# oleg-savchenko/jax_nbody_emulator_with_dj

Measured on AMD Instinct MI355X. Metric: voxels/sec (disp+vel) on 512^3 box, ndiv=4, higher is better.
Workload: dtype f32-equivalent: f16x3 split MFMA (3 f16 MFMAs per product, f32 accumulate)

## Files before the change

### jax_nbody_emulator_with_dj_amd/csrc/nbe_engine.cpp

```cpp

#include "../../include/nbe.h"
#include "nbe_kernels.h"

#include <sched.h>

#include <cmath>
#include <cstdarg>
#include <cstdio>
#include <cstdlib>
#include <cstring>
#include <algorithm>
#include <atomic>
#include <chrono>
#include <condition_variable>
#include <deque>
#include <map>
#include <memory>
#include <mutex>
#include <string>
#include <thread>
#include <vector>

using namespace nbe;

// ... 1239 lines not shown
    if (d.k != 3) return fail("%s/%s: conv layers have k=3", d.block, d.layer);
    *kind = 0;
    return 0;
}

static int expected_shape(nbe_ctx* c, const std::string& blk, const std::string& lay, int* cout, int* cin) {
    const int m = c->mid;
    int bi, bo;
    if (blk == "conv_l00") { bi = c->in_chan; bo = m; }
    else if (blk == "conv_r2" || blk == "conv_r1" || blk == "conv_r00") { bi = 2 * m; bo = m; }
    else if (blk == "conv_r01") { bi = m; bo = c->out_chan; }
    else { bi = m; bo = m; }
    const int midc = bi > bo ? bi : bo;
    if (lay == "skip") { *cin = bi; *cout = bo; }
    else if (blk.rfind("down_", 0) == 0 || blk.rfind("up_", 0) == 0) { *cin = bi; *cout = bo; }
    else if (lay == "conv_0") { *cin = bi; *cout = midc; }
    else if (lay == "conv_1") { *cin = midc; *cout = bo; }
    else return fail("unknown layer %s/%s", blk.c_str(), lay.c_str());
    return 0;
}

static const char* kBlocks[15] = {"conv_l00", "conv_l01", "down_l0", "conv_l1", "down_l1", "conv_l2", "down_l2", "conv_c",
                                  "up_r2", "conv_r2", "up_r1", "conv_r1", "up_r0", "conv_r00", "conv_r01"};

static int pack_wino(nbe_ctx* c) {
    c->wino_ok = false;
    if (!((c->prec == PREC_F16X3 && (c->vel ? c->gauge_active : true)) || (c->prec == PREC_F16 && c->vel && c->gauge_active))) return 0;
    if (!c->wino_flag) HIPCHK(hipMalloc((void**)&c->wino_flag, 4));
    HIPCHK(hipMemsetAsync(c->wino_flag, 0, 4, c->stream));
    for (auto& kv : c->layers) {
        Layer& L = kv.second;
        if (L.pw.ww && L.kind == 0 && (L.g6 || !c->vel)) launch_pack_h3w(L.wn, L.cout, L.cin, L.pw.cin_pad, L.pw.ctiles, L.pw.ww, c->wino_flag, c->stream, c->prec);
        if (L.pw.ww && L.kind == 1 && (c->vel ? (L.b_sub && c->fuse) : c->novel_fuse)) {
            launch_pack_h3w_skip(L.wn, L.cout, L.cin, L.pw, L.pw.ww, c->wino_flag, c->stream);
            if (c->vel) launch_pack_h3w_skip(c->prec == PREC_F16 ? L.dwn_f : L.dwn, L.cout, L.cin, L.pw, L.pw.ww + L.pw.floats, c->wino_flag, c->stream);
        }
    }
    int bad = 0;
    HIPCHK(hipMemcpyAsync(&bad, c->wino_flag, 4, hipMemcpyDeviceToHost, c->stream));
    HIPCHK(hipStreamSynchronize(c->stream));
    c->wino_ok = bad == 0;
    if (!c->vel) c->fuse = c->novel_fuse && c->wino_ok;
    if (c->prec == PREC_F16) c->fuse = c->fuse && c->wino_ok;
    return 0;
}

static int wire_novel(nbe_ctx* c) {
    c->novel_fuse = false;
    if (c->vel || c->prec != PREC_F16X3) return 0;
    for (const char* b : kBlocks) {
        if (!strncmp(b, "down_", 5) || !strncmp(b, "up_", 3)) continue;
        auto i1 = c->layers.find(std::string(b) + "/conv_1"), is = c->layers.find(std::string(b) + "/skip");
        if (i1 == c->layers.end() || is == c->layers.end()) return fail("internal: block %s", b);
        Layer &L1 = i1->second, &Ls = is->second;
        if (!L1.pw.ww || !Ls.pw.ww || 2 * (Ls.pw.cin_pad / 16) > 16 || L1.pw.ctiles != Ls.pw.ctiles) return 0;
    }
    for (const char* b : kBlocks) {
        if (!strncmp(b, "down_", 5) || !strncmp(b, "up_", 3)) continue;
        Layer &L1 = c->layers[std::string(b) + "/conv_1"], &Ls = c->layers[std::string(b) + "/skip"];
        L1.fskip = &Ls;
        const int nb = L1.pw.ctiles * 32 * L1.pw.ni;
        HIPCHK(hipMalloc((void**)&L1.bias_f, nb * 4));
    }
    c->novel_fuse = true;
    return 0;
}

static int wire_gauge(nbe_ctx* c) {
// ... 162 lines not shown
        int ec, ei;
        if (expected_shape(c, L.block, L.layer, &ec, &ei)) return 1;
        if (ec != d.cout || ei != d.cin)
            return fail("%s/%s: weight shape (%d,%d,k) does not match the architecture (%d,%d,k)", d.block, d.layer, d.cout, d.cin, ec, ei);
        L.first = (L.block == "conv_l00") && (L.layer == "conv_0" || L.layer == "skip");
        const size_t nw = (size_t)d.cout * d.cin * d.k * d.k * d.k;
        PackedW& pw = L.pw;
        pw.mode = L.kind == 0 ? MODE_FLAT3 : (L.kind == 2 ? MODE_DOWN : MODE_FLAT1);
        pw.prec = c->prec;
        pw.ni = (prec_is_half(c->prec) || d.cout > 32) ? 2 : 1;
        pw.cin = d.cin; pw.cout = d.cout;
        pw.cin_pad = roundup(d.cin, prec_ck(c->prec, pw.mode));
        pw.ctiles = (d.cout + 32 * pw.ni - 1) / (32 * pw.ni);
        pw.nsets = L.kind == 3 ? 8 : 1;
        pw.floats = (int64_t)pw.ctiles * 32 * pw.ni * mode_nseg(pw.mode) * mode_taps(pw.mode) * pw.cin_pad / (c->prec == PREC_F16 ? 2 : 1);
        HIPCHK(hipMalloc((void**)&pw.w, pw.floats * pw.nsets * 4));
        if (c->vel) HIPCHK(hipMalloc((void**)&pw.dw, pw.floats * pw.nsets * 4));
        const int nb = pw.ctiles * 32 * pw.ni;
        HIPCHK(hipMalloc((void**)&pw.bias, nb * 4));
        HIPCHK(hipMemset(pw.bias, 0, nb * 4));
        HIPCHK(hipMemcpy(pw.bias, d.bias, d.cout * 4, hipMemcpyHostToDevice));
        if (c->prec == PREC_F16X3 && c->vel && (L.kind == 0 || L.kind == 1) && d.cout <= 4 && !L.first) {
            PackedW& pn = L.pwn;
            pn = pw; pn.w = nullptr; pn.dw = nullptr;
            pn.cout_t = 16; pn.ctiles = 1;
            pn.floats = (int64_t)16 * mode_nseg(pn.mode) * mode_taps(pn.mode) * pn.cin_pad;
            HIPCHK(hipMalloc((void**)&pn.w, pn.floats * 4));
            if (L.kind == 1) HIPCHK(hipMalloc((void**)&pn.dw, pn.floats * 4));
        }
        if ((c->prec == PREC_F16X3 && L.kind == 0 && !L.first && !L.pwn.w && pw.cin_pad / 16 <= 8) ||
            (L.kind == 0 && !L.first && wino_f16_layer(c->prec, c->vel, pw.cin_pad)))
            HIPCHK(hipMalloc((void**)&pw.ww, pw.floats * 4 / 3 * 4));
        if (c->prec == PREC_F16X3 && L.kind == 1 && !L.pwn.w && pw.cin_pad / 16 <= 8)
            HIPCHK(hipMalloc((void**)&pw.ww, pw.floats * 2 * 4));
        if (style && L.kind == 1 && !L.first && wino_f16_layer(c->prec, c->vel, pw.cin_pad)) {
            HIPCHK(hipMalloc((void**)&pw.ww, pw.floats * 2 * 4));
            HIPCHK(hipMalloc((void**)&L.dwn_f, nw * 4));
        }
        if (prec_is_half(c->prec) && L.kind == 0 && L.first && d.cin <= 3 && d.cout <= 64)
            HIPCHK(hipMalloc((void**)&pw.stem, 4 * 3 * 4 * 64 * 16));
        HIPCHK(hipMalloc((void**)&L.bias0, nb * 4));
        HIPCHK(hipMemcpy(L.bias0, pw.bias, nb * 4, hipMemcpyDeviceToDevice));
        for (int i = 0; i < d.cout; ++i)
            if (std::isfinite(d.bias[i])) c->bias_max = std::max(c->bias_max, std::fabs(d.bias[i]));
        HIPCHK(hipMalloc((void**)&L.wn, nw * 4));
        if (c->vel) HIPCHK(hipMalloc((void**)&L.dwn, nw * 4));
        if (style) {
            if (!d.style_weight || !d.style_bias) return fail("%s/%s: style_weight and style_bias are required", d.block, d.layer);
            HIPCHK(hipMalloc((void**)&L.weight, nw * 4));
            HIPCHK(hipMalloc((void**)&L.sw, d.cin * 2 * 4));
            HIPCHK(hipMalloc((void**)&L.sb, d.cin * 4));
            HIPCHK(hipMemcpy(L.weight, d.weight, nw * 4, hipMemcpyHostToDevice));
            HIPCHK(hipMemcpy(L.sw, d.style_weight, d.cin * 2 * 4, hipMemcpyHostToDevice));
            HIPCHK(hipMemcpy(L.sb, d.style_bias, d.cin * 4, hipMemcpyHostToDevice));
        } else {
            if (c->vel && !d.dweight) return fail("%s/%s: dweight is required for premodulated velocity weights", d.block, d.layer);
            HIPCHK(hipMemcpy(L.wn, d.weight, nw * 4, hipMemcpyHostToDevice));
            if (c->vel) HIPCHK(hipMemcpy(L.dwn, d.dweight, nw * 4, hipMemcpyHostToDevice));
            launch_pack(L.wn, d.cout, d.cin, L.kind, pw, pw.w, c->stream);
            if (c->vel) launch_pack(L.dwn, d.cout, d.cin, L.kind, pw, pw.dw, c->stream);
            if (L.pwn.w) launch_pack(L.wn, d.cout, d.cin, L.kind, L.pwn, L.pwn.w, c->stream);
            if (L.pwn.dw) launch_pack(L.dwn, d.cout, d.cin, L.kind, L.pwn, L.pwn.dw, c->stream);
        }
        c->layers[L.block + "/" + L.layer] = L;
    }
    for (const char* b : kBlocks) {
        const bool rs = !strncmp(b, "down_", 5) || !strncmp(b, "up_", 3);
// ... 1217 lines not shown
```

### jax_nbody_emulator_with_dj_amd/csrc/nbe_kernels.h

```cpp
#pragma once
#include <hip/hip_runtime.h>
#include <stdint.h>

namespace nbe {

struct Planes {
    float* x = nullptr;
    float* dx = nullptr;
    int64_t pstride = 0;
    int G = 0;
    int D = 0, H = 0, W = 0;
    int64_t vox() const { return (int64_t)D * H * W; }
};

enum Precision { PREC_F32 = 0, PREC_F16X3 = 1, PREC_F16 = 2 };
inline constexpr bool prec_is_half(int prec) { return prec == PREC_F16X3 || prec == PREC_F16; }
inline constexpr int prec_parts(int prec) { return prec == PREC_F16X3 ? 2 : 1; }
constexpr float H3_SCALE = 2048.0f, H3_INV = 1.0f / 2048.0f;
constexpr int H3_RANGE_UP = 6;

constexpr int NBE_MAX_GROUPS = 64;

enum ConvMode { MODE_FLAT3 = 0, MODE_FLAT1 = 1, MODE_DOWN = 2 };
enum ConvFlags { F_ACT = 1, F_RES = 2, F_SKIP_NODX = 4 };
// ... 24 lines not shown
    Planes in;
    int64_t in_off = 0;
    int Dv = 0, Hv = 0, Wv = 0;
    Planes out;
    int out_g0 = 0;
    int osz = 1, oz = 0, oy = 0, ox = 0;
    Planes res;
    int flags = 0;
    int set = 0;
    const float* gout = nullptr;
    const float* beta = nullptr;
    const float* bias = nullptr;
    Planes in2;
    int csplit_ch = 0;
    Planes sk, sk2;
    int sk_split_ch = 0;
    int64_t sk_off = 0;
    const PackedW* skw = nullptr;
    bool wino = false;
};

int launch_conv(const PackedW& pw, const ConvLaunch& L, bool vel, bool has_dx, hipStream_t s);

void launch_modulate(const float* weight, const float* style_weight, const float* style_bias,
                     int cout, int cin, int k3, float s0, float s1, float eps, int first_layer,
                     float* w_n, float* dw_tot , hipStream_t s,
                     const float* a_in = nullptr, float* beta_out = nullptr, const float* b_sub = nullptr);
void launch_style_alpha(const float* style_weight, const float* style_bias, int cin, float s0, float s1,
                        float* alpha, int* flag, hipStream_t s);
void launch_pack(const float* w_oidhw, int cout, int cin, int kind, const PackedW& pw, float* dst, hipStream_t s);

void launch_pack_h3w(const float* w_oidhw, int cout, int cin, int cin_pad, int ctiles, float* dst, int* flag, hipStream_t s,
                     int prec = PREC_F16X3);
void launch_pack_h3w_skip(const float* w_oidhw, int cout, int cin, const PackedW& pw, float* dst, int* flag, hipStream_t s);

void launch_gather(const float* box, int C, int Db, int Hb, int Wb, int a0, int a1, int a2,
                   const Planes& dst, float scale, int prec, hipStream_t s);
void launch_to_planes(const float* src, int C, const Planes& dst, bool tangent, float scale, int prec, hipStream_t s);
void launch_from_planes(const Planes& src, bool tangent, int C, float* dst, int prec, hipStream_t s);
void launch_crop(const Planes& src, int c, const Planes& dst, int g0, bool vel, hipStream_t s, int cz = -1);
struct HeadScale { float k_disp = 6.f, k_dy = 0.f, k_x0 = 0.f; int* bad = nullptr; };
void launch_head(const Planes& y, const Planes& xin, int c0, int C, const HeadScale& hs, bool vel,
                 void* disp, void* velo, int out_dtype, int Db, int Hb, int Wb, int a0, int a1, int a2,
                 int prec, hipStream_t s, int pad = 0);
void launch_absmax(const float* src, int64_t n, unsigned* out_bits, hipStream_t s);
void launch_zero(void* dst, int64_t bytes, hipStream_t s);
void launch_scale(const float* src, float* dst, int n, float f, hipStream_t s, const float* src2 = nullptr);

void launch_fill_yx(const Planes& t, int pad, bool vel, hipStream_t s);
void launch_wrap_pad(const Planes& src, const Planes& dst, int pad, bool vel, hipStream_t s, int padz = 0);

void launch_tag_word(unsigned* dst, unsigned v, const unsigned* expect_at, unsigned* flag, unsigned bit, hipStream_t s);

struct ProbeLaunch {
    const float* x; int64_t pstride; int H, W, g0, prec, C;
    int ext[3], org[3], per[3];
    int zlo, zhi, zper;
    int o[3], n, nw;
    unsigned* bits; unsigned* count;
};
void launch_probe_signs(const ProbeLaunch& a, hipStream_t s);

void h3q_read_stamps(double* out16, hipStream_t s);

}
```

### jax_nbody_emulator_with_dj_amd/csrc/nbe_kernels_h3.hip

```cpp

#include "nbe_kernels_internal.h"
#include <cstdlib>
#include <cstdio>
#include <algorithm>

#ifndef NBE_DBG
#define NBE_DBG 0
#endif

namespace nbe {

extern __shared__ __attribute__((aligned(16))) f32x4 lds_h3[];

__device__ __forceinline__ void split4(const f32x4 v, half4& hi, half4& lo) {
#pragma unroll
    for (int e = 0; e < 4; ++e) {
        hi[e] = (_Float16)v[e];
        lo[e] = (_Float16)__builtin_fmaf((float)hi[e], -H3_SCALE, v[e] * H3_SCALE);
    }
}
__device__ __forceinline__ f32x4 join4(const half4 hi, const half4 lo) {
    f32x4 v;
#pragma unroll
    for (int e = 0; e < 4; ++e) v[e] = (float)hi[e] + (float)lo[e] * H3_INV;
// ... 1825 lines not shown
    const int nstage = nseg * nchunk;
    long r = idx;
    const int j = (int)(r % 8); r /= 8;
    const int co = (int)(r % cout_t); r /= cout_t;
    const int un = 2 * parts;
    const int u = (int)(r % un); r /= un;
    const int tap = (int)(r % TAPS); r /= TAPS;
    const int stage = (int)(r % nstage); r /= nstage;
    const long per_set_ct = halves_per_set / ((long)nstage * TAPS * un * cout_t * 8);
    const int ct = (int)(r % per_set_ct); r /= per_set_ct;
    const int set = (int)r;
    const int chunk = stage / nseg, seg = stage - chunk * nseg;
    const int h = u / parts, part = u - h * parts;
    const int ci = f16w ? chunk * 32 + 8 * u + j : chunk * 16 + 8 * h + j;
    const int oc = ct * cout_t + co;
    int k, kz, ky, kx;
    if (kind == 0) { k = 3; kz = seg / 3; ky = seg % 3; kx = tap; }
    else if (kind == 1) { k = 1; kz = ky = kx = 0; }
    else if (kind == 2) { k = 2; kz = seg >> 2; ky = (seg >> 1) & 1; kx = seg & 1; }
    else { k = 2; kz = 1 - ((set >> 2) & 1); ky = 1 - ((set >> 1) & 1); kx = 1 - (set & 1); }
    float v = 0.f;
    if (oc < cout && ci < cin) v = w[(((size_t)oc * cin + ci) * k + kz) * k * k + ky * k + kx];
    if (wscale != 0.f) {
        v *= wscale;
        if (!(fabsf(v) <= 60000.f)) { atomicOr(flag, 1); v = 0.f; }
        const _Float16 h = (_Float16)v;
        dst[idx] = (part == 0 || f16w) ? h : (_Float16)(v - (float)h);
        return;
    }
    const _Float16 hi = (_Float16)v;
    dst[idx] = part == 0 ? hi : (_Float16)((v - (float)hi) * H3_SCALE);
}

void launch_pack_h3w_skip(const float* w_oidhw, int cout, int cin, const PackedW& pw, float* dst, int* flag, hipStream_t s) {
    const long halves = pw.floats * 2;
    if (pw.prec == PREC_F16) {
        hipLaunchKernelGGL(pack_h3_kernel, dim3((unsigned)((halves + 255) / 256)), dim3(256), 0, s, w_oidhw, cout, cin,
                           1, pw.mode, pw.cin_pad / 32, halves, 1, 2, pw.cout_t, (_Float16*)dst, 256.0f, flag, 1);
        return;
    }
    hipLaunchKernelGGL(pack_h3_kernel, dim3((unsigned)((halves + 255) / 256)), dim3(256), 0, s, w_oidhw, cout, cin,
                       1, pw.mode, pw.cin_pad / 16, halves, 1, 2, pw.cout_t, (_Float16*)dst, 16384.0f, flag);
}

void launch_pack_h3(const float* w_oidhw, int cout, int cin, int kind, const PackedW& pw, float* dst, hipStream_t s) {
    if (pw.stem && kind == 0 && (dst == pw.w || dst == pw.dw)) {
        const int parts = pw.prec == PREC_F16X3 ? 2 : 1;
        hipLaunchKernelGGL(pack_stem_kernel, dim3(48), dim3(256), 0, s, w_oidhw, cout, cin,
                           (_Float16*)pw.stem + (dst == pw.dw ? parts * 3 * 4 * 64 * 8 : 0), parts);
    }
    const long halves = pw.floats * 2;
    const long total = halves * pw.nsets;
    hipLaunchKernelGGL(pack_h3_kernel, dim3((unsigned)((total + 255) / 256)), dim3(256), 0, s, w_oidhw, cout, cin,
                       kind, pw.mode, pw.cin_pad / 16, halves, pw.nsets, pw.prec == PREC_F16X3 ? 2 : 1, pw.cout_t,
                       (_Float16*)dst);
}

__device__ __forceinline__ half8 ld8(const float* base, long plane, long pstride, long v) {
    return *(const half8*)(base + (plane * pstride + v) * 4);
}
__device__ __forceinline__ float join1(const half8& hi, const half8& lo, int e, int parts) {
    return parts == 2 ? (float)hi[e] + (float)lo[e] * H3_INV : (float)hi[e];
}

__global__ __launch_bounds__(256) void gather_h8_kernel(const float* __restrict__ box, int C, int Db, int Hb, int Wb,
                                                        int a0, int a1, int a2, float* __restrict__ dst, long pstride,
                                                        int G, int D, int H, int W, float scale, int parts) {
    const long v = (long)blockIdx.x * blockDim.x + threadIdx.x;
    const long V = (long)D * H * W;
    if (v >= V) return;
    const int z = (int)(v / ((long)H * W)), rem = (int)(v - (long)z * H * W);
    const int y = rem / W, x = rem - y * W;
    const int bz = ((a0 + z) % Db + Db) % Db, by = ((a1 + y) % Hb + Hb) % Hb, bx = ((a2 + x) % Wb + Wb) % Wb;
    const long bo = ((long)bz * Hb + by) * Wb + bx;
    const long bstride = (long)Db * Hb * Wb;
// ... 100 lines not shown
```

### jax_nbody_emulator_with_dj_amd/csrc/nbe_kernels_wino.h

```cpp

#ifndef NBE_EPI_MAX
#define NBE_EPI_MAX 1
#endif
#ifndef NBE_WINO_ZROW
#define NBE_WINO_ZROW 1
#endif
#ifndef NBE_WINO_ITEMREG
#define NBE_WINO_ITEMREG 1
#endif
#ifndef NBE_WINO_LOU
#define NBE_WINO_LOU (NBE_XF_F32 ? 0 : 1)
#endif
constexpr int NBE_MAX_WSTAGES = 32;
constexpr int NBE_MAX_WSKIP = 16;
constexpr float WINO_WSCALE = 16384.0f;
constexpr float WINO_WSCALE_F16 = 256.0f;

struct WinoSrc { const char* xa; const char* xb; long dxd; const char* w; long psb; float sb; int pad_; };

struct WinoKArgs {
    int H, W, Dv, Hv, Wv, Ho, Wo;
    int nchunk, cout_groups, flags, ntiles, tny, tnx;
    int zblock;
    float* y; float* dy; long out_pstride; int out_g0;
    const float* bias; const float* gout; const float* beta;
    const float* r; const float* dr; long res_pstride;
    float inv_scale;
    int nskip;
    long dws_delta;
    WinoSrc st[NBE_MAX_WSTAGES + NBE_MAX_WSKIP];
};

template <bool SKIP, bool NOVEL, bool F16 = false>
__global__ __launch_bounds__(512, 2) void conv_h3w_kernel(WinoKArgs a) {
    static_assert(!(F16 && NOVEL), "the float16 form has no displacement-only variant");
    typedef HGGeom<false> G;
    constexpr int NW = 8, CT = 64, TAPU = G::TAPU, WGU = G::WG, XBASE = G::XBASE, MT = 4, NT = 2, NTILE = 8;
    constexpr int ZROW = G::LDS_UNITS;
    f32x4* lds = lds_h3;
    const half8* L8 = (const half8*)lds_h3;
    half8* L8w = (half8*)lds_h3;
    const int tid = threadIdx.x;
    const int lane = tid & 63;
    const int wave = __builtin_amdgcn_readfirstlane(tid >> 6);
    const int c = lane & 15, q = lane >> 4, kh = q & 1, ks = q >> 1;

    const int nct = (a.cout_groups + 7) / 8;
    const int vt = xcd_tile(blockIdx.x, a.ntiles * nct);
    const int tile = vt / nct, ct = vt - tile * nct;
    const int npair = a.Dv >> 1;
    int zp, ty, tx;
    {
        const int zb = a.zblock;
        const int full = (npair / zb) * zb;
        const int per_blk = zb * a.tny * a.tnx;
        if (tile < (npair / zb) * per_blk) {
            const int blk = tile / per_blk, r = tile - blk * per_blk;
            const int zi = r % zb, tyx = r / zb;
            zp = blk * zb + zi; ty = tyx / a.tnx; tx = tyx - ty * a.tnx;
        } else {
            const int r = tile - (npair / zb) * per_blk, rem = npair - full;
            const int zi = r % rem, tyx = r / rem;
            zp = full + zi; ty = tyx / a.tnx; tx = tyx - ty * a.tnx;
        }
    }
    const int y0 = ty * (NOVEL ? 2 * HP_ROWS : HP_ROWS), x0 = tx * HP_COLS, z0 = 2 * zp;
    const int nst = 4 * a.nchunk;

    const long to = (((long)z0 * a.H + y0) * a.W + x0) * 16;
    const long wcm = (long)ct * nst * WGU * 16, wcs = (long)ct * a.nskip * TAPU * 16;

    struct Nxt { const char *xa, *xb, *w0; long dxd, psb; float sb; } nx;
    auto set_next = [&](int s) {
        const WinoSrc e = a.st[s];
        nx.xa = e.xa + to; nx.xb = e.xb + to; nx.dxd = e.dxd; nx.psb = e.psb; nx.w0 = e.w + (SKIP && s >= nst ? wcs : wcm); nx.sb = e.sb;
    };
    unsigned lane16 = (unsigned)lane << 4;
    asm volatile("" : "+v"(lane16));
    auto dma_w = [&](int buf, int t) {
        const int n = wave + NW * t;
        unsigned l16 = (unsigned)lane;
        if (NBE_WINO_ZROW && !F16) l16 = lane16;
        else asm volatile("v_lshlrev_b32 %0, 4, %0" : "+v"(l16));
        if (n < G::NWI) dma16s(nx.w0 + (long)n * 1024, l16, lds + buf * WGU + n * 64);
    };
    auto dma_raw = [&](int buf) {
        unsigned l16 = (unsigned)lane;
        asm volatile("v_lshlrev_b32 %0, 4, %0" : "+v"(l16));
        dma16s(nx.w0 + (wave < 4 ? 0 : a.dws_delta) + (long)(wave & 3) * 1024, l16, lds + buf * WGU + wave * 64);
#pragma unroll
        for (int t = 0; t < 6; ++t) {
            const int tensor = t / 3, n = wave + NW * (t % 3), pl = n / 6, k = n - 6 * pl;
            const int u = k * 64 + lane;
            const int uu = u < HP_PL ? u : HP_PL - 1;
            const int row = (uu * 241) >> 13, col = uu - row * HP_RS;
            if (u < HP_PL)
                dma16s(nx.xa + (tensor ? nx.dxd : 0) + (long)pl * nx.psb, (unsigned)(row * a.W + col) * 16u,
                       lds + XBASE + buf * HQ_XB + tensor * HQ_XT + pl * HQ_PP + k * 64);
        }
    };
    constexpr bool ITEMREG = NBE_WINO_ITEMREG && !F16;
    int it_uu[3] = {0, 0, 0};
    unsigned it_go[3] = {0u, 0u, 0u};
    if (ITEMREG) {
#pragma unroll
        for (int j = 0; j < 3; ++j) {
            const int u = ((wave + NW * j) % 6) * 64 + lane;
            it_uu[j] = u < HP_PL ? u : HP_PL - 1;
            const int row = (it_uu[j] * 241) >> 13, col = it_uu[j] - row * HP_RS;
            it_go[j] = (unsigned)(row * a.W + col) * 16u;
        }
#pragma unroll
        for (int j = 0; j < 3; ++j) asm volatile("" : "+v"(it_uu[j]), "+v"(it_go[j]));
    }
    auto item_unit = [&](int j, bool& valid) {
        if (ITEMREG) {
            valid = lane < HP_PL - ((wave + NW * j) % 6) * 64;
            return it_uu[j];
        }
        int l = lane;
        asm volatile("" : "+v"(l));
        const int u = ((wave + NW * j) % 6) * 64 + l;
        valid = u < HP_PL;
        return valid ? u : HP_PL - 1;
    };
    auto item_goff_j = [&](int j) {
        if (ITEMREG) return it_go[j];
        bool v;
        const int uu = item_unit(j, v);
        const int row = (uu * 241) >> 13, col = uu - row * HP_RS;
        return (unsigned)(row * a.W + col) * 16u;
// ... 230 lines not shown
        {
            const _Float16 m1 = ks ? kInv : (_Float16)1.0f;
#pragma unroll
            for (int mt = 0; mt < MT; ++mt) a1[mt] = a1[mt] * m1;
        }
        NBE_SB; MM8(Y, a1, b1x, -1, 0, false, true); NBE_SB;
#endif
#if NBE_WINO_ZROW
        LA(a2, ks ? ZROW + c : aS + CT);
#else
        LA(a2, aS + CT);
#endif
        LB(xl, xb + SH5 + bP32 + HQ_PP);
        NBE_SB; MM8(DY, a1, b1d, -1, 0, false); NBE_SB;
        LB(xh, xb + SH5 + bP32); LA(wh, wb + 5 * TAPU + aP);
#if NBE_WINO_ZROW
        NBE_SB; MM8(Y, a2, b1x, -1, 0, false); NBE_SB;
#else
#pragma unroll
        for (int mt = 0; mt < MT; ++mt) a2[mt] = ks ? zero : a2[mt];
        NBE_SB; MM8(Y, a2, b1x, -1, 0, false, true); NBE_SB;
#endif
        MM8(DY, a2, b1d, -1, 0, false); NBE_SB;
        }
        pair(Y, DY, -1, nb, px, wb + 5 * TAPU, xb + SH5 + bP32,
             [&] { LB(xl, xb + SH7 + bP1 + HQ_PP); }, [&] { LA(wh, wb + 7 * TAPU + aP); }, [&] { LB(xh, xb + SH7 + bP1); },
             none, px, hk, [&] { if (px) { st_write(1, nb, xf); st_load(2, g); } });
        pair(Y, DY, -1, nb, px, wb + 7 * TAPU, xb + SH7 + bP1,
             [&] { if (pre) LB(xl, xbn + bP1 + HQ_PP); }, [&] { if (pre) LA(wh, wbn + aP); }, [&] { if (pre) LB(xh, xbn + bP1); },
             [&] { asm volatile("s_waitcnt vmcnt(0) lgkmcnt(0)\n\ts_barrier" ::: "memory"); },
             px, hk, [&] { if (px) st_write(2, nb, xf); });
    };

    auto raw_stage = [&](f32x4 (&Y)[NTILE], f32x4 (&DY)[NTILE], int s, bool px) {
        if (px) set_next(s + 1);
        int par = s & 1;
        asm volatile("" : "+s"(par));
        int nb = 1 - par;
        asm volatile("" : "+s"(nb));
        const int wb = par * WGU, xb = XBASE + par * HQ_XB;
        if (px) dma_raw(nb);
        half8 a1[MT], a2[MT], d1[MT], d2[MT], bx[NT], bd[NT];
        const half8 zero = {0, 0, 0, 0, 0, 0, 0, 0};
        const _Float16 m1 = ks ? kInv : (_Float16)1.0f;
        const int aS = wb + (2 * kh) * CT + c;
        const int bS = xb + (2 * kh + ks) * HQ_PP + rowp * HP_RS + c + SH4;
        if (F16) {
            const int aF = wb + (2 * kh + ks) * CT + c;
            LA(a1, aF); LB(bx, bS); LB(bd, bS + HQ_XT); LA(d1, aF + TAPU);
            NBE_SB; MM8(Y, a1, bx, -1, 0, false); NBE_SB;
            MM8(DY, a1, bd, -1, 0, false); NBE_SB;
            MM8(DY, d1, bx, -1, 0, false); NBE_SB;
            asm volatile("s_waitcnt vmcnt(0) lgkmcnt(0)\n\ts_barrier" ::: "memory");
            return;
        }
        LA(a1, aS); LB(bx, bS); LA(a2, aS + CT); LB(bd, bS + HQ_XT);
#pragma unroll
        for (int mt = 0; mt < MT; ++mt) a1[mt] = a1[mt] * m1;
        NBE_SB; MM8(Y, a1, bx, -1, 0, false, true); NBE_SB;
        if (!NOVEL) LA(d1, aS + TAPU);
#pragma unroll
        for (int mt = 0; mt < MT; ++mt) a2[mt] = ks ? zero : a2[mt];
        NBE_SB; MM8(Y, a2, bx, -1, 0, false, true); NBE_SB;
        if (!NOVEL) LA(d2, aS + TAPU + CT);
        if (NOVEL || !(a.flags & F_SKIP_NODX)) {
            NBE_SB; MM8(DY, a1, bd, -1, 0, false); NBE_SB;
            MM8(DY, a2, bd, -1, 0, false); NBE_SB;
        }
        if (!NOVEL) {
#pragma unroll
            for (int mt = 0; mt < MT; ++mt) { d1[mt] = d1[mt] * m1; d2[mt] = ks ? zero : d2[mt]; }
            NBE_SB; MM8(DY, d1, bx, -1, 0, false, true); NBE_SB;
            MM8(DY, d2, bx, -1, 0, false, true); NBE_SB;
        }
        asm volatile("s_waitcnt vmcnt(0) lgkmcnt(0)\n\ts_barrier" ::: "memory");
    };

    {
        if (NBE_WINO_ZROW && !F16 && tid < 64) L8w[ZROW + tid] = half8{0, 0, 0, 0, 0, 0, 0, 0};
        set_next(0);
#pragma unroll
        for (int k = 0; k < G::NWS; ++k) dma_w(0, k);
        {
            Stg g0, g1, g2;
            st_load(0, g0); st_load(1, g1); st_load(2, g2);
            st_store(0, 0, g0); st_store(1, 0, g1); st_store(2, 0, g2);
        }
        asm volatile("s_waitcnt vmcnt(0) lgkmcnt(0)" ::: "memory");
        __syncthreads();
        LA(wh, aP); LB(xl, XBASE + bP1 + HQ_PP); LB(xh, XBASE + bP1);
    }

    auto butterfly = [&] {
            asm volatile("s_nop 15\n\ts_nop 15" ::: "memory");
#pragma unroll
            for (int t = 0; t < NTILE; ++t) {
                f32x4 p, m;
#pragma unroll
                for (int e = 0; e < 4; ++e) { p[e] = acc_read(YA[t][e]); m[e] = acc_read(YB[t][e]); }
                YA[t] = p + m; YB[t] = p - m;
                asm volatile("" : "+a"(YA[t]), "+a"(YB[t]));
                __builtin_amdgcn_sched_barrier(0);
#pragma unroll
                for (int e = 0; e < 4; ++e) { p[e] = acc_read(DA[t][e]); m[e] = acc_read(DB[t][e]); }
                DA[t] = p + m; DB[t] = p - m;
                asm volatile("" : "+a"(DA[t]), "+a"(DB[t]));
                __builtin_amdgcn_sched_barrier(0);
            }
            asm volatile("s_nop 7" ::: "memory");
            LA(wh, aP); LB(xl, XBASE + bP1 + HQ_PP); LB(xh, XBASE + bP1);
    };
    const int npairs = 2 * a.nchunk;
    for (int s2 = 0; s2 + 1 < npairs; ++s2) {
        if (s2 == a.nchunk) butterfly();
        stage(YA, DA, 2 * s2, std::integral_constant<int, 1>());
        stage(YB, DB, 2 * s2 + 1, std::integral_constant<int, 1>());
    }
    if (npairs - 1 == a.nchunk) butterfly();
    stage(YA, DA, 2 * npairs - 2, std::integral_constant<int, 1>());
    stage(YB, DB, 2 * npairs - 1, std::integral_constant<int, SKIP ? 2 : 0>());
    if (SKIP) {
        for (int sc = 0; sc < a.nskip; ++sc) {
            raw_stage(YA, DA, nst + 2 * sc, true);
            raw_stage(YB, DB, nst + 2 * sc + 1, sc + 1 < a.nskip);
        }
    }
#undef NBE_SB
#undef SNAKE
    asm volatile("s_nop 15\n\ts_nop 15" ::: "memory");

    const bool act = a.flags & F_ACT, gauge = !NOVEL && a.gout != nullptr;
    f32x4 bv[MT], be[MT], gv[MT];
    int unit[MT];
    bool uok[MT];
#pragma unroll
    for (int mt = 0; mt < MT; ++mt) {
        unit[mt] = ct * (CT / 8) + 2 * mt + ks;
        uok[mt] = unit[mt] < a.cout_groups;
        if (!uok[mt]) unit[mt] = a.cout_groups - 1;
        bv[mt] = *(const f32x4*)(a.bias + unit[mt] * 8 + 4 * kh);
        be[mt] = f32x4{0.f, 0.f, 0.f, 0.f};
        if (!NOVEL) be[mt] = *(const f32x4*)(a.beta + unit[mt] * 8 + 4 * kh);
        gv[mt] = f32x4{0.f, 0.f, 0.f, 0.f};
        if (!NOVEL && gauge) gv[mt] = *(const f32x4*)(a.gout + unit[mt] * 8 + 4 * kh);
    }
#pragma unroll
    for (int mt = 0; mt < MT; ++mt) asm volatile("" : "+v"(bv[mt]), "+v"(be[mt]), "+v"(gv[mt]));
    long ob_mt[MT];
#pragma unroll
    for (int mt = 0; mt < MT; ++mt) ob_mt[mt] = (long)(a.out_g0 + (F16 ? 1 : 2) * unit[mt]) * a.out_pstride * 16 + 8 * kh;
    const long ol_off = a.out_pstride * 16;
    auto epilogue = [&](f32x4 (&Y)[NTILE], f32x4 (&DY)[NTILE], int z) {
        int o[NT];
        bool ook[NT], ook2[NT];
#pragma unroll
        for (int nt = 0; nt < NT; ++nt) {
            const int yy = y0 + rowp, xx = x0 + 16 * nt + c;
            ook[nt] = yy < a.Hv && xx < a.Wv;
// ... 86 lines not shown
            }
        }
    };
    epilogue(YA, DA, z0);
    epilogue(YB, DB, z0 + 1);
}

__global__ __launch_bounds__(256) void pack_h3w_kernel(const float* __restrict__ w, int cout, int cin, int nchunk, long total,
                                                       _Float16* __restrict__ dst, int* __restrict__ flag, int f16) {
    const long idx = (long)blockIdx.x * blockDim.x + threadIdx.x;
    if (idx >= total) return;
    long r = idx;
    const int j = (int)(r % 8); r /= 8;
    const int co = (int)(r % 64); r /= 64;
    const int u = (int)(r % 4); r /= 4;
    const int tap = (int)(r % 9); r /= 9;
    const int stage = (int)(r % (4 * nchunk)); r /= 4 * nchunk;
    const int ct = (int)r;
    const int chunk = stage >> 2, xi = stage & 3;
    const int h = u >> 1, part = u & 1;
    const int ci = f16 ? chunk * 32 + 8 * u + j : chunk * 16 + 8 * h + j, oc = ct * 64 + co;
    float v = 0.f;
    if (oc < cout && ci < cin) {
        const float* p = w + (((size_t)oc * cin + ci) * 3) * 9 + tap;
        const float w0 = p[0], w1 = p[9], w2 = p[18];
        v = xi == 0 ? w0 : xi == 1 ? 0.5f * (w0 + w1 + w2) : xi == 2 ? 0.5f * (w0 - w1 + w2) : -w2;
    }
    v *= f16 ? WINO_WSCALE_F16 : WINO_WSCALE;
    if (!(fabsf(v) <= 60000.f)) { atomicOr(flag, 1); v = 0.f; }
    const _Float16 hi = (_Float16)v;
    dst[idx] = (part == 0 || f16) ? hi : (_Float16)(v - (float)hi);
}

void launch_pack_h3w(const float* w_oidhw, int cout, int cin, int cin_pad, int ctiles, float* dst, int* flag, hipStream_t s, int prec) {
    const bool f16 = prec == PREC_F16;
    const int nchunk = cin_pad / (f16 ? 32 : 16);
    const long total = (long)ctiles * 4 * nchunk * 9 * 4 * 64 * 8;
    hipLaunchKernelGGL(pack_h3w_kernel, dim3((unsigned)((total + 255) / 256)), dim3(256), 0, s, w_oidhw, cout, cin, nchunk, total,
                       (_Float16*)dst, flag, f16 ? 1 : 0);
}

static int launch_h3w(const ConvKArgs& ka_in, const float* ww, const float* wws, long wws_set_floats, int ctiles, hipStream_t s,
                      bool novel = false, bool f16 = false) {
    typedef HGGeom<false> G;
    constexpr size_t smem = (size_t)(G::LDS_UNITS + 64) * 16;
    static_assert(smem <= 160 * 1024, "LDS budget of one CU");
    ConvKArgs ka = ka_in;
    if (f16) {
        if (novel || (ka.nchunk & 1) || (ka.csplit < ka.nchunk && (ka.csplit & 1))) return 1;
        if (ka.nskip > 0 && ((ka.nskip & 1) || (ka.s_csplit < ka.nskip && (ka.s_csplit & 1)) || (ka.flags & F_SKIP_NODX))) return 1;
        ka.nchunk /= 2; if (ka.csplit < (1 << 29)) ka.csplit /= 2;
        ka.nskip /= 2; if (ka.s_csplit < (1 << 29)) ka.s_csplit /= 2;
    }
    if (!ww || (!f16 && (ka.flags & F_RES)) || (ka.Dv & 1) || 4 * ka.nchunk > NBE_MAX_WSTAGES || (!novel && !ka.beta)) return 1;
    if (ka.nskip > 0 && (!wws || 2 * ka.nskip > NBE_MAX_WSKIP)) return 1;
    if (ctiles != (ka.cout_groups + 7) / 8) return 1;
    if (std::max(ka.in_pstride, ka.csplit < ka.nchunk ? ka.in2_pstride : 0L) * 16 + 16L * (HP_ROWS + 2) * ka.W >= (1L << 32) - (1L << 20)) return 1;
    WinoKArgs wa;
    wa.H = ka.H; wa.W = ka.W; wa.Dv = ka.Dv; wa.Hv = ka.Hv; wa.Wv = ka.Wv; wa.Ho = ka.Ho; wa.Wo = ka.Wo;
    wa.nchunk = ka.nchunk; wa.cout_groups = ka.cout_groups; wa.flags = ka.flags;
    const int trows = novel ? 2 * HP_ROWS : HP_ROWS;
    wa.tny = (ka.Hv + trows - 1) / trows;
    wa.tnx = (ka.Wv + HP_COLS - 1) / HP_COLS;
    wa.ntiles = (ka.Dv / 2) * wa.tny * wa.tnx;
    wa.y = ka.y; wa.dy = ka.dy; wa.out_pstride = ka.out_pstride; wa.out_g0 = ka.out_g0;
    wa.bias = ka.bias; wa.gout = novel ? nullptr : ka.gout; wa.beta = novel ? nullptr : ka.beta;
    const long rows8 = (long)HP_ROWS * ka.W * 16;
    wa.inv_scale = 1.0f / (f16 ? WINO_WSCALE_F16 : WINO_WSCALE);
    wa.r = ka.r; wa.dr = ka.dr; wa.res_pstride = ka.res_pstride;
    wa.zblock = std::min(8, ka.Dv / 2);
    wa.nskip = ka.nskip; wa.dws_delta = wws_set_floats * 4;
    static const int XI[2][2] = {{1, 2}, {0, 3}};
    static const int PA[4] = {0, 1, 2, 1}, PB[4] = {2, 2, 1, 3};
    static const float SB[4] = {-1.f, 1.f, -1.f, -1.f};
    const long plane = (long)ka.H * ka.W * 16;
    for (int ph = 0; ph < 2; ++ph)
        for (int chunk = 0; chunk < ka.nchunk; ++chunk)
            for (int ab = 0; ab < 2; ++ab) {
                const int xi = XI[ph][ab];
                const bool second = chunk >= ka.csplit;
                const long ps = second ? ka.in2_pstride : ka.in_pstride;
                const char* x = (const char*)(second ? ka.x2 : ka.x);
                const char* dx = (const char*)(second ? ka.dx2 : ka.dx);
                const long off = (long)(second ? chunk - ka.csplit : chunk) * 4 * ps * 16;
                WinoSrc& e = wa.st[(ph * ka.nchunk + chunk) * 2 + ab];
                e.xa = x + off + PA[xi] * plane; e.xb = x + off + PB[xi] * plane; e.dxd = novel ? rows8 : dx - x;
                e.w = (const char*)ww + (long)(chunk * 4 + xi) * G::WG * 16; e.psb = ps * 16; e.sb = SB[xi]; e.pad_ = 0;
            }
    for (int sc = 0; sc < ka.nskip; ++sc)
        for (int ab = 0; ab < 2; ++ab) {
            const bool second = sc >= ka.s_csplit;
            const long ps = second ? ka.s2_pstride : ka.s_pstride;
            const char* x = (const char*)(second ? ka.xs2 : ka.xs);
            const char* dx = (const char*)(second ? ka.dxs2 : ka.dxs);
            const long off = (long)(second ? sc - ka.s_csplit : sc) * 4 * ps * 16 + ab * plane;
            WinoSrc& e = wa.st[4 * ka.nchunk + 2 * sc + ab];
            e.xa = x + off; e.xb = e.xa; e.dxd = novel ? rows8 : dx - x; e.w = (const char*)wws + (long)sc * G::TAPU * 16; e.psb = ps * 16; e.sb = 0.f; e.pad_ = 0;
        }
    const bool skip = ka.nskip > 0;
    if (novel) wa.dws_delta = 0;
    auto kern = f16 ? (skip ? conv_h3w_kernel<true, false, true> : conv_h3w_kernel<false, false, true>)
              : novel ? (skip ? conv_h3w_kernel<true, true> : conv_h3w_kernel<false, true>)
              : (skip ? conv_h3w_kernel<true, false> : conv_h3w_kernel<false, false>);
    ensure_lds_limit((const void*)kern, smem);
    dim3 grid(wa.ntiles * ctiles, 1, 1), block(512, 1, 1);
    hipLaunchKernelGGL(kern, grid, block, smem, s, wa);
    return 0;
}
```

Before: 98.06 million.

## Merge skip-path raw stages into one stage covering both z-slices per weight load

The fused Winograd conv kernel's skip (1x1) raw phase previously ran two stages per skip chunk, one per z-slice, each reloading weights. It now loads both z-slices of input into the two LDS buffers in one stage and reuses the same weight fragments for both accumulators. Weights are repacked by a new pack kernel that pre-splits the hi/lo halves and pre-applies the scale factor, so the per-lane multiply and zeroing work is gone. This halves the number of skip stages and barriers, at the cost of a larger packed weight buffer (3x floats instead of 2x) and a more complex DMA layout that must fit in the existing LDS buffers.

```diff
diff --git a/jax_nbody_emulator_with_dj_amd/csrc/nbe_engine.cpp b/jax_nbody_emulator_with_dj_amd/csrc/nbe_engine.cpp
--- a/jax_nbody_emulator_with_dj_amd/csrc/nbe_engine.cpp
+++ b/jax_nbody_emulator_with_dj_amd/csrc/nbe_engine.cpp
@@ -1295,8 +1295,8 @@
         Layer& L = kv.second;
         if (L.pw.ww && L.kind == 0 && (L.g6 || !c->vel)) launch_pack_h3w(L.wn, L.cout, L.cin, L.pw.cin_pad, L.pw.ctiles, L.pw.ww, c->wino_flag, c->stream, c->prec);
         if (L.pw.ww && L.kind == 1 && (c->vel ? (L.b_sub && c->fuse) : c->novel_fuse)) {
-            launch_pack_h3w_skip(L.wn, L.cout, L.cin, L.pw, L.pw.ww, c->wino_flag, c->stream);
-            if (c->vel) launch_pack_h3w_skip(c->prec == PREC_F16 ? L.dwn_f : L.dwn, L.cout, L.cin, L.pw, L.pw.ww + L.pw.floats, c->wino_flag, c->stream);
+            launch_pack_h3w_skip(L.wn, L.cout, L.cin, L.pw, 0, c->wino_flag, c->stream);
+            if (c->vel) launch_pack_h3w_skip(c->prec == PREC_F16 ? L.dwn_f : L.dwn, L.cout, L.cin, L.pw, 1, c->wino_flag, c->stream);
         }
     }
     int bad = 0;
@@ -1525,7 +1525,7 @@
             (L.kind == 0 && !L.first && wino_f16_layer(c->prec, c->vel, pw.cin_pad)))
             HIPCHK(hipMalloc((void**)&pw.ww, pw.floats * 4 / 3 * 4));
         if (c->prec == PREC_F16X3 && L.kind == 1 && !L.pwn.w && pw.cin_pad / 16 <= 8)
-            HIPCHK(hipMalloc((void**)&pw.ww, pw.floats * 2 * 4));
+            HIPCHK(hipMalloc((void**)&pw.ww, pw.floats * 3 * 4));
         if (style && L.kind == 1 && !L.first && wino_f16_layer(c->prec, c->vel, pw.cin_pad)) {
             HIPCHK(hipMalloc((void**)&pw.ww, pw.floats * 2 * 4));
             HIPCHK(hipMalloc((void**)&L.dwn_f, nw * 4));
diff --git a/jax_nbody_emulator_with_dj_amd/csrc/nbe_kernels.h b/jax_nbody_emulator_with_dj_amd/csrc/nbe_kernels.h
--- a/jax_nbody_emulator_with_dj_amd/csrc/nbe_kernels.h
+++ b/jax_nbody_emulator_with_dj_amd/csrc/nbe_kernels.h
@@ -80,7 +80,7 @@
 
 void launch_pack_h3w(const float* w_oidhw, int cout, int cin, int cin_pad, int ctiles, float* dst, int* flag, hipStream_t s,
                      int prec = PREC_F16X3);
-void launch_pack_h3w_skip(const float* w_oidhw, int cout, int cin, const PackedW& pw, float* dst, int* flag, hipStream_t s);
+void launch_pack_h3w_skip(const float* w_oidhw, int cout, int cin, const PackedW& pw, int set, int* flag, hipStream_t s);
 
 void launch_gather(const float* box, int C, int Db, int Hb, int Wb, int a0, int a1, int a2,
                    const Planes& dst, float scale, int prec, hipStream_t s);
diff --git a/jax_nbody_emulator_with_dj_amd/csrc/nbe_kernels_h3.hip b/jax_nbody_emulator_with_dj_amd/csrc/nbe_kernels_h3.hip
--- a/jax_nbody_emulator_with_dj_amd/csrc/nbe_kernels_h3.hip
+++ b/jax_nbody_emulator_with_dj_amd/csrc/nbe_kernels_h3.hip
@@ -1881,15 +1881,14 @@
     dst[idx] = part == 0 ? hi : (_Float16)((v - (float)hi) * H3_SCALE);
 }
 
-void launch_pack_h3w_skip(const float* w_oidhw, int cout, int cin, const PackedW& pw, float* dst, int* flag, hipStream_t s) {
+void launch_pack_h3w_skip(const float* w_oidhw, int cout, int cin, const PackedW& pw, int set, int* flag, hipStream_t s) {
     const long halves = pw.floats * 2;
     if (pw.prec == PREC_F16) {
         hipLaunchKernelGGL(pack_h3_kernel, dim3((unsigned)((halves + 255) / 256)), dim3(256), 0, s, w_oidhw, cout, cin,
-                           1, pw.mode, pw.cin_pad / 32, halves, 1, 2, pw.cout_t, (_Float16*)dst, 256.0f, flag, 1);
+                           1, pw.mode, pw.cin_pad / 32, halves, 1, 2, pw.cout_t, (_Float16*)(pw.ww + set * pw.floats), 256.0f, flag, 1);
         return;
     }
-    hipLaunchKernelGGL(pack_h3_kernel, dim3((unsigned)((halves + 255) / 256)), dim3(256), 0, s, w_oidhw, cout, cin,
-                       1, pw.mode, pw.cin_pad / 16, halves, 1, 2, pw.cout_t, (_Float16*)dst, 16384.0f, flag);
+    launch_pack_h3w_skip_x3(w_oidhw, cout, cin, pw.cin_pad, pw.ctiles, set, pw.ww, flag, s);
 }
 
 void launch_pack_h3(const float* w_oidhw, int cout, int cin, int kind, const PackedW& pw, float* dst, hipStream_t s) {
diff --git a/jax_nbody_emulator_with_dj_amd/csrc/nbe_kernels_wino.h b/jax_nbody_emulator_with_dj_amd/csrc/nbe_kernels_wino.h
--- a/jax_nbody_emulator_with_dj_amd/csrc/nbe_kernels_wino.h
+++ b/jax_nbody_emulator_with_dj_amd/csrc/nbe_kernels_wino.h
@@ -28,8 +28,15 @@
     float inv_scale;
     int nskip;
     long dws_delta;
-    WinoSrc st[NBE_MAX_WSTAGES + NBE_MAX_WSKIP];
+    long raw_plane;
+    WinoSrc st[NBE_MAX_WSTAGES + NBE_MAX_WSKIP / 2];
 };
+
+constexpr int WRAW_P = HP_ROWS * HP_COLS;
+constexpr int WRAW_T = 4 * WRAW_P;
+constexpr int WRAW_W = 2 * WRAW_T;
+constexpr int WRAW_WU = 12 * 64;
+static_assert(WRAW_W + 4 * 64 <= HGGeom<false>::WG && WRAW_W + 8 * 64 <= HQ_XB, "the raw phase fits the transformed phase's buffers");
 
 template <bool SKIP, bool NOVEL, bool F16 = false>
 __global__ __launch_bounds__(512, 2) void conv_h3w_kernel(WinoKArgs a) {
@@ -68,7 +75,7 @@
     const int nst = 4 * a.nchunk;
 
     const long to = (((long)z0 * a.H + y0) * a.W + x0) * 16;
-    const long wcm = (long)ct * nst * WGU * 16, wcs = (long)ct * a.nskip * TAPU * 16;
+    const long wcm = (long)ct * nst * WGU * 16, wcs = (long)ct * a.nskip * (F16 ? TAPU : WRAW_WU) * 16;
 
     struct Nxt { const char *xa, *xb, *w0; long dxd, psb; float sb; } nx;
     auto set_next = [&](int s) {
@@ -84,19 +91,31 @@
         else asm volatile("v_lshlrev_b32 %0, 4, %0" : "+v"(l16));
         if (n < G::NWI) dma16s(nx.w0 + (long)n * 1024, l16, lds + buf * WGU + n * 64);
     };
+    auto raw_piece = [&](int buf, int j) {
+        const int wbR = buf * WGU, xbR = XBASE + buf * HQ_XB;
+        if (j >= 8) {
+            const int n = wave + NW * (j - 8);
+            unsigned l16 = (unsigned)lane;
+            asm volatile("v_lshlrev_b32 %0, 4, %0" : "+v"(l16));
+            if (F16) {
+                if (j == 8) dma16s(nx.w0 + (n < 4 ? 0 : a.dws_delta) + (long)(n & 3) * 1024, l16,
+                                   lds + (n < 4 ? wbR + WRAW_W + n * 64 : xbR + WRAW_W + 128 + (n - 4) * 64));
+            } else if (n < (NOVEL ? 6 : 12))
+                dma16s(nx.w0 + (long)n * 1024, l16, lds + (n < 4 ? wbR + WRAW_W + n * 64 : xbR + WRAW_W + (n - 4) * 64));
+            return;
+        }
+        const int z = j >> 2, tensor = (j >> 1) & 1, pl = (j & 1) * 2 + (wave >> 2), k = wave & 3;
+        int l = lane;
+        asm volatile("" : "+v"(l));
+        const unsigned go = (unsigned)((2 * k + (l >> 5) + 1) * a.W + (l & 31) + 1) * 16u;
+        dma16s(nx.xa + (tensor ? nx.dxd : 0) + (z ? a.raw_plane : 0) + (long)pl * nx.psb, go,
+               lds + (z ? xbR : wbR) + tensor * WRAW_T + pl * WRAW_P + k * 64);
+    };
     auto dma_raw = [&](int buf) {
-        unsigned l16 = (unsigned)lane;
-        asm volatile("v_lshlrev_b32 %0, 4, %0" : "+v"(l16));
-        dma16s(nx.w0 + (wave < 4 ? 0 : a.dws_delta) + (long)(wave & 3) * 1024, l16, lds + buf * WGU + wave * 64);
-#pragma unroll
-        for (int t = 0; t < 6; ++t) {
-            const int tensor = t / 3, n = wave + NW * (t % 3), pl = n / 6, k = n - 6 * pl;
-            const int u = k * 64 + lane;
-            const int uu = u < HP_PL ? u : HP_PL - 1;
-            const int row = (uu * 241) >> 13, col = uu - row * HP_RS;
-            if (u < HP_PL)
-                dma16s(nx.xa + (tensor ? nx.dxd : 0) + (long)pl * nx.psb, (unsigned)(row * a.W + col) * 16u,
-                       lds + XBASE + buf * HQ_XB + tensor * HQ_XT + pl * HQ_PP + k * 64);
+        raw_piece(buf, 8); raw_piece(buf, 9);
+        raw_piece(buf, 0); raw_piece(buf, 1); raw_piece(buf, 4); raw_piece(buf, 5);
+        if (NOVEL || F16 || !(a.flags & F_SKIP_NODX)) {
+            raw_piece(buf, 2); raw_piece(buf, 3); raw_piece(buf, 6); raw_piece(buf, 7);
         }
     };
     constexpr bool ITEMREG = NBE_WINO_ITEMREG && !F16;
@@ -393,52 +412,67 @@
              px, hk, [&] { if (px) st_write(2, nb, xf); });
     };
 
-    auto raw_stage = [&](f32x4 (&Y)[NTILE], f32x4 (&DY)[NTILE], int s, bool px) {
+    auto raw_stage = [&](int s, bool px) {
         if (px) set_next(s + 1);
         int par = s & 1;
         asm volatile("" : "+s"(par));
         int nb = 1 - par;
         asm volatile("" : "+s"(nb));
         const int wb = par * WGU, xb = XBASE + par * HQ_XB;
-        if (px) dma_raw(nb);
-        half8 a1[MT], a2[MT], d1[MT], d2[MT], bx[NT], bd[NT];
-        const half8 zero = {0, 0, 0, 0, 0, 0, 0, 0};
-        const _Float16 m1 = ks ? kInv : (_Float16)1.0f;
-        const int aS = wb + (2 * kh) * CT + c;
-        const int bS = xb + (2 * kh + ks) * HQ_PP + rowp * HP_RS + c + SH4;
+        half8 a1[MT], a2[MT], d1[MT], d2[MT], bx[NT], bd[NT], bx2[NT], bd2[NT];
+        const int pB = (2 * kh + ks) * WRAW_P + rowp * HP_COLS + c;
+        const int bS = wb + pB, bS2 = xb + pB;
+        const int aS = wb + WRAW_W + (2 * kh + ks) * CT + c;
         if (F16) {
-            const int aF = wb + (2 * kh + ks) * CT + c;
-            LA(a1, aF); LB(bx, bS); LB(bd, bS + HQ_XT); LA(d1, aF + TAPU);
-            NBE_SB; MM8(Y, a1, bx, -1, 0, false); NBE_SB;
-            MM8(DY, a1, bd, -1, 0, false); NBE_SB;
-            MM8(DY, d1, bx, -1, 0, false); NBE_SB;
+            LA(a1, aS); LB(bx, bS); LB(bd, bS + WRAW_T); LA(d1, xb + WRAW_W + 128 + (2 * kh + ks) * CT + c);
+            if (px) dma_raw(nb);
+            NBE_SB; MM8(YA, a1, bx, -1, 0, false); NBE_SB;
+            MM8(DA, a1, bd, -1, 0, false); NBE_SB;
+            LB(bd2, bS2 + WRAW_T);
+            NBE_SB; MM8(DA, d1, bx, -1, 0, false); NBE_SB;
+            LB(bx2, bS2);
+            NBE_SB; MM8(DB, a1, bd2, -1, 0, false); NBE_SB;
+            MM8(YB, a1, bx2, -1, 0, false); NBE_SB;
+            MM8(DB, d1, bx2, -1, 0, false); NBE_SB;
             asm volatile("s_waitcnt vmcnt(0) lgkmcnt(0)\n\ts_barrier" ::: "memory");
             return;
         }
-        LA(a1, aS); LB(bx, bS); LA(a2, aS + CT); LB(bd, bS + HQ_XT);
-#pragma unroll
-        for (int mt = 0; mt < MT; ++mt) a1[mt] = a1[mt] * m1;
-        NBE_SB; MM8(Y, a1, bx, -1, 0, false, true); NBE_SB;
-        if (!NOVEL) LA(d1, aS + TAPU);
-#pragma unroll
-        for (int mt = 0; mt < MT; ++mt) a2[mt] = ks ? zero : a2[mt];
-        NBE_SB; MM8(Y, a2, bx, -1, 0, false, true); NBE_SB;
-        if (!NOVEL) LA(d2, aS + TAPU + CT);
-        if (NOVEL || !(a.flags & F_SKIP_NODX)) {
-            NBE_SB; MM8(DY, a1, bd, -1, 0, false); NBE_SB;
-            MM8(DY, a2, bd, -1, 0, false); NBE_SB;
-        }
+        const bool dxs = NOVEL || !(a.flags & F_SKIP_NODX);
+        const int aL = ks ? ZROW + c : xb + WRAW_W + kh * CT + c;
+        const int dS = xb + WRAW_W + 128 + (2 * kh + ks) * CT + c;
+        const int dL = ks ? ZROW + c : xb + WRAW_W + 384 + kh * CT + c;
+        LA(a1, aS); LB(bx, bS); LA(a2, aL);
+        if (dxs) LB(bd, bS + WRAW_T);
+        if (px) dma_raw(nb);
+        NBE_SB; MM8(YA, a1, bx, -1, 0, false); NBE_SB;
+        if (!NOVEL) LA(d1, dS);
+        NBE_SB; MM8(YA, a2, bx, -1, 0, false); NBE_SB;
+        if (!NOVEL) LA(d2, dL);
+        if (dxs) {
+            NBE_SB; MM8(DA, a1, bd, -1, 0, false); NBE_SB;
+            MM8(DA, a2, bd, -1, 0, false); NBE_SB;
+            LB(bd2, bS2 + WRAW_T);
+        } else LB(bx2, bS2);
         if (!NOVEL) {
-#pragma unroll
-            for (int mt = 0; mt < MT; ++mt) { d1[mt] = d1[mt] * m1; d2[mt] = ks ? zero : d2[mt]; }
-            NBE_SB; MM8(DY, d1, bx, -1, 0, false, true); NBE_SB;
-            MM8(DY, d2, bx, -1, 0, false, true); NBE_SB;
+            NBE_SB; MM8(DA, d1, bx, -1, 0, false); NBE_SB;
+            MM8(DA, d2, bx, -1, 0, false); NBE_SB;
+        }
+        if (dxs) LB(bx2, bS2);
+        if (dxs) {
+            NBE_SB; MM8(DB, a1, bd2, -1, 0, false); NBE_SB;
+            MM8(DB, a2, bd2, -1, 0, false); NBE_SB;
+        }
+        MM8(YB, a1, bx2, -1, 0, false); NBE_SB;
+        MM8(YB, a2, bx2, -1, 0, false); NBE_SB;
+        if (!NOVEL) {
+            MM8(DB, d1, bx2, -1, 0, false); NBE_SB;
+            MM8(DB, d2, bx2, -1, 0, false); NBE_SB;
         }
         asm volatile("s_waitcnt vmcnt(0) lgkmcnt(0)\n\ts_barrier" ::: "memory");
     };
 
     {
-        if (NBE_WINO_ZROW && !F16 && tid < 64) L8w[ZROW + tid] = half8{0, 0, 0, 0, 0, 0, 0, 0};
+        if ((NBE_WINO_ZROW || SKIP) && !F16 && tid < 64) L8w[ZROW + tid] = half8{0, 0, 0, 0, 0, 0, 0, 0};
         set_next(0);
 #pragma unroll
         for (int k = 0; k < G::NWS; ++k) dma_w(0, k);
@@ -481,10 +515,7 @@
     stage(YA, DA, 2 * npairs - 2, std::integral_constant<int, 1>());
     stage(YB, DB, 2 * npairs - 1, std::integral_constant<int, SKIP ? 2 : 0>());
     if (SKIP) {
-        for (int sc = 0; sc < a.nskip; ++sc) {
-            raw_stage(YA, DA, nst + 2 * sc, true);
-            raw_stage(YB, DB, nst + 2 * sc + 1, sc + 1 < a.nskip);
-        }
+        for (int sc = 0; sc < a.nskip; ++sc) raw_stage(nst + sc, sc + 1 < a.nskip);
     }
 #undef NBE_SB
 #undef SNAKE
@@ -637,6 +668,34 @@
     dst[idx] = (part == 0 || f16) ? hi : (_Float16)(v - (float)hi);
 }
 
+__global__ __launch_bounds__(256) void pack_h3w_skip_kernel(const float* __restrict__ w, int cout, int cin, int nchunk, long total,
+                                                            _Float16* __restrict__ dst, int set, int* __restrict__ flag) {
+    const long idx = (long)blockIdx.x * blockDim.x + threadIdx.x;
+    if (idx >= total) return;
+    long r = idx;
+    const int j = (int)(r % 8); r /= 8;
+    const int co = (int)(r % 64); r /= 64;
+    const int u = (int)(r % 6); r /= 6;
+    const int chunk = (int)(r % nchunk); r /= nchunk;
+    const int ct = (int)r;
+    const int kh = u < 4 ? u >> 1 : u - 4;
+    const int ci = chunk * 16 + 8 * kh + j, oc = ct * 64 + co;
+    float v = 0.f;
+    if (oc < cout && ci < cin) v = w[(size_t)oc * cin + ci];
+    v *= WINO_WSCALE;
+    if (!(fabsf(v) <= 60000.f)) { atomicOr(flag, 1); v = 0.f; }
+    const _Float16 hi = (_Float16)v;
+    const _Float16 out = u >= 4 ? (_Float16)(v - (float)hi) : (u & 1) ? hi * (_Float16)H3_INV : hi;
+    dst[((((long)ct * nchunk + chunk) * 2 + set) * 6 + u) * 512 + co * 8 + j] = out;
+}
+
+void launch_pack_h3w_skip_x3(const float* w_oidhw, int cout, int cin, int cin_pad, int ctiles, int set, float* dst, int* flag, hipStream_t s) {
+    const int nchunk = cin_pad / 16;
+    const long total = (long)ctiles * nchunk * 6 * 64 * 8;
+    hipLaunchKernelGGL(pack_h3w_skip_kernel, dim3((unsigned)((total + 255) / 256)), dim3(256), 0, s, w_oidhw, cout, cin, nchunk, total,
+                       (_Float16*)dst, set, flag);
+}
+
 void launch_pack_h3w(const float* w_oidhw, int cout, int cin, int cin_pad, int ctiles, float* dst, int* flag, hipStream_t s, int prec) {
     const bool f16 = prec == PREC_F16;
     const int nchunk = cin_pad / (f16 ? 32 : 16);
@@ -674,7 +733,7 @@
     wa.inv_scale = 1.0f / (f16 ? WINO_WSCALE_F16 : WINO_WSCALE);
     wa.r = ka.r; wa.dr = ka.dr; wa.res_pstride = ka.res_pstride;
     wa.zblock = std::min(8, ka.Dv / 2);
-    wa.nskip = ka.nskip; wa.dws_delta = wws_set_floats * 4;
+    wa.nskip = ka.nskip; wa.dws_delta = wws_set_floats * 4; wa.raw_plane = (long)ka.H * ka.W * 16;
     static const int XI[2][2] = {{1, 2}, {0, 3}};
     static const int PA[4] = {0, 1, 2, 1}, PB[4] = {2, 2, 1, 3};
     static const float SB[4] = {-1.f, 1.f, -1.f, -1.f};
@@ -692,18 +751,16 @@
                 e.xa = x + off + PA[xi] * plane; e.xb = x + off + PB[xi] * plane; e.dxd = novel ? rows8 : dx - x;
                 e.w = (const char*)ww + (long)(chunk * 4 + xi) * G::WG * 16; e.psb = ps * 16; e.sb = SB[xi]; e.pad_ = 0;
             }
-    for (int sc = 0; sc < ka.nskip; ++sc)
-        for (int ab = 0; ab < 2; ++ab) {
-            const bool second = sc >= ka.s_csplit;
-            const long ps = second ? ka.s2_pstride : ka.s_pstride;
-            const char* x = (const char*)(second ? ka.xs2 : ka.xs);
-            const char* dx = (const char*)(second ? ka.dxs2 : ka.dxs);
-            const long off = (long)(second ? sc - ka.s_csplit : sc) * 4 * ps * 16 + ab * plane;
-            WinoSrc& e = wa.st[4 * ka.nchunk + 2 * sc + ab];
-            e.xa = x + off; e.xb = e.xa; e.dxd = novel ? rows8 : dx - x; e.w = (const char*)wws + (long)sc * G::TAPU * 16; e.psb = ps * 16; e.sb = 0.f; e.pad_ = 0;
-        }
+    for (int sc = 0; sc < ka.nskip; ++sc) {
+        const bool second = sc >= ka.s_csplit;
+        const long ps = second ? ka.s2_pstride : ka.s_pstride;
+        const char* x = (const char*)(second ? ka.xs2 : ka.xs);
+        const char* dx = (const char*)(second ? ka.dxs2 : ka.dxs);
+        const long off = (long)(second ? sc - ka.s_csplit : sc) * 4 * ps * 16;
+        WinoSrc& e = wa.st[4 * ka.nchunk + sc];
+        e.xa = x + off; e.xb = e.xa; e.dxd = novel ? rows8 : dx - x; e.w = (const char*)wws + (long)sc * (f16 ? G::TAPU : WRAW_WU) * 16; e.psb = ps * 16; e.sb = 0.f; e.pad_ = 0;
+    }
     const bool skip = ka.nskip > 0;
-    if (novel) wa.dws_delta = 0;
     auto kern = f16 ? (skip ? conv_h3w_kernel<true, false, true> : conv_h3w_kernel<false, false, true>)
               : novel ? (skip ? conv_h3w_kernel<true, true> : conv_h3w_kernel<false, true>)
               : (skip ? conv_h3w_kernel<true, false> : conv_h3w_kernel<false, false>);
```

Result: no change. 98.93 million, median of 6 (+0.9%).
